# FlinkML/flink-parameter-server

Hardware: NVIDIA H100
Metric: matrix-factorization updates/sec (whole box, max over ranks) (higher is better)
Workload: dtype fp32

## Files before the change

flink-parameter-server_b200/models/mf/device.py:

```python
from __future__ import annotations

import math
import os
from typing import Iterable, Optional, Sequence, Tuple

import torch
import torch.distributed as dist

from ...errors import FactorIsNotANumberException
from ...ops import native
from ...utils.metrics import GLOBAL as METRICS
from ...runtime.device_stream import DevicePrefetcher
from ...store.replica_cache import ReplicaCache
from ...store.sharded_table import ShardedTable

ERR_SIGMOID = 0
ERR_PLAIN = 1

DEFAULT_DEVICE_PULL_LIMIT = 0

L2_TABLE_BYTES = 48 << 20
WINDOW_BUDGET = 256 << 20
WINDOW_BYTES_PER_ROW = 8 + 12
WINDOW_MAX_STRIDE = 128
# ... 89 lines not shown
                 output_ring=None, loss: str = "pointwise", regularization: float = 0.0,
                 step_window: Optional[int] = None, optimizer: str = "sgd",
                 negative_sampling: str = "uniform", margin: Optional[float] = None):
        self._pending = []
        self.step_window = 0
        check_negative_sampling(negative_sampling, negative_sample_rate)
        self.negative_sampling = negative_sampling
        if loss not in ("pointwise", "bpr", "warp"):
            raise ValueError(f"loss must be 'pointwise', 'bpr' or 'warp', got {loss!r}")
        self.loss, self.reg = loss, float(regularization)
        if loss == "pointwise" and self.reg != 0.0:
            raise ValueError("regularization is only supported with loss='bpr' or loss='warp'")
        self.margin = check_warp(loss, margin, optimizer=optimizer, negative_sampling=negative_sampling)
        if loss != "pointwise":
            if output_ring is not None:
                raise ValueError(f"the per-update output ring is not supported with loss={loss!r}")
            if kernel == "tma":
                raise ValueError(f"kernel='tma' is not supported with loss={loss!r}")
            if item_blocking:
                raise ValueError(f"item_blocking is not supported with loss={loss!r}")
            item_blocking = False
        self.device = torch.cuda.current_device() if device is None else int(device)
        self.cuda_device = torch.device("cuda", self.device)
        self.group = group
        ready = dist.is_available() and dist.is_initialized()
        self.world = dist.get_world_size(group) if ready else 1
        self.rank = dist.get_rank(group) if ready else 0
        if item_cache is None:
            item_cache = self.world > 1 and os.environ.get("FPS_ITEM_CACHE", "1") != "0"
        check_optimizer(optimizer, item_cache=bool(item_cache), output_ring=output_ring, kernel=kernel)
        self.optimizer = optimizer
        self.num_users, self.num_items, self.k = int(num_users), int(num_items), int(num_factors)
        self.lr = float(learning_rate)
        self.neg = int(negative_sample_rate)
        self.pull_limit = int(pull_limit)
        self.err_mode = int(err_mode)
        self.seed = int(seed)
        self.step_no = 0
        self.kernel = kernel
        self.credits = (torch.tensor([self.pull_limit, 0], dtype=torch.int32, device=self.cuda_device)
                        if self.pull_limit >= 32 and os.environ.get("FPS_STATIC_LIMITER", "0") != "1"
                        and loss == "pointwise" and optimizer == "sgd" else None)
        self.output_ring = output_ring
        with torch.cuda.device(self.device):
            self._items = ShardedTable(num_items, num_factors, partition="hash", group=group,
                                      device=self.device, init="uniform",
                                      init_range=(range_min, range_max), seed=seed * 2 + 1,
                                      track_touched=track_touched)
            n_local = -(-self.num_users // self.world)
            self._users = torch.empty((n_local, self._items.stride), dtype=torch.float32,
                                     device=self.cuda_device)
            native.init_rows(self._users, self.k, self.rank, self.world, native.PART_HASH, n_local,
                             seed * 2 + 2, range_min, range_max)
            self._stats = torch.zeros(STATS_SIZE[loss], dtype=torch.float32, device=self.cuda_device)
            self._user_acc = self._item_acc = None
            if optimizer == "adagrad":
                self._user_acc = torch.zeros(n_local, dtype=torch.float32, device=self.cuda_device)
                self._item_acc = self._items.row_accumulators()
            self._nan_flag = torch.zeros(1, dtype=torch.int32, device=self.cuda_device)
            self.user_memory = int(user_memory) if self.neg > 0 else 0
            if self.user_memory > 0:
                self.seen = torch.full((n_local, self.user_memory), -1, dtype=torch.int32,
                                       device=self.cuda_device)
                self.seen_pos = torch.zeros(n_local, dtype=torch.int32, device=self.cuda_device)
            self._registry = (native.seen_registry(self.num_items, self.cuda_device)
                              if negative_sampling == "seen" else None)
        self.item_cache = bool(item_cache)
        self.sync_every = max(1, int(sync_every))
        self.sync_interval_ms = sync_interval_ms
        self.flush_count, self.flush_require = flush_count, flush_require
        self._own_inplace = replica_own_inplace
        self.replica = (ReplicaCache(self._items, self.sync_every, sync_interval_ms,
                                     require=flush_require, flush_count=flush_count,
                                     own_inplace=replica_own_inplace)
                        if self.item_cache else None)
        row_bytes = self._items.stride * 4
        if item_blocking is None:
            item_blocking = ((self.world == 1 or self.item_cache) and self.num_items * row_bytes > (48 << 20)
                             and (self.neg == 0 or self.user_memory > 0 or negative_sampling == "seen")
                             and os.environ.get("FPS_ITEM_BLOCKING", "1") != "0")
        self.item_blocking = bool(item_blocking)
        block_bytes = int(os.environ.get("FPS_BLOCK_BYTES", block_bytes))
        self.l2_hints = self.item_blocking and os.environ.get("FPS_L2_HINTS", "0") == "1"
        per_bucket = max(1, int(block_bytes) // row_bytes)
        self.block_shift = max(0, per_bucket.bit_length() - 1)
        table_rows = self._items.rows_per_shard * self.world if self.item_cache else self.num_items
        self._table_rows = table_rows
        while -(-table_rows >> self.block_shift) > native.BUCKET_MAX:
            self.block_shift += 1
        self.block_buckets = max(1, -(-table_rows >> self.block_shift))
        if self.item_blocking:
            with torch.cuda.device(self.device):
                self._bucket_scratch = torch.zeros(2 * native.BUCKET_MAX, dtype=torch.int32,
                                                   device=self.cuda_device)
        self.step_window = step_window_size(step_window, world=self.world, item_cache=self.item_cache,
                                            loss=self.loss, table_rows=self.num_items, stride=self._items.stride,
                                            env=os.environ.get("FPS_STEP_WINDOW"), optimizer=optimizer)
        self._win = None
        self._win_phase_ns = None
        self._graph_capture = False
        self._per_launch = False
        self._items.barrier()

    @property
    def stats(self) -> torch.Tensor:
        self._drain()
        return self._stats

    @property
    def users(self) -> torch.Tensor:
        self._drain()
        return self._users

    @property
    def items(self) -> ShardedTable:
        self._drain()
        return self._items

    @property
    def nan_flag(self) -> torch.Tensor:
        self._drain()
        return self._nan_flag

    @property
    def accumulators(self) -> Optional[Tuple[torch.Tensor, torch.Tensor]]:
        self._drain()
        if self._item_acc is None:
            return None
        return self._user_acc, self._item_acc.local

    def _windowable(self, users, items, ratings) -> bool:
        if self.step_window < 2 or self._graph_capture or self._per_launch:
            return False
        packed = items is None
        return step_windowable(
            neg=self.neg, output_ring=self.output_ring, pull_limit=self.pull_limit, credits=self.credits,
            kernel=self.kernel, kernel_env=os.environ.get("FPS_MF_KERNEL", "reg"),
            reg_variant_env=os.environ.get("FPS_MF_REG_VARIANT"), l2_hints=self.l2_hints, packed=packed,
            dtypes=(users.dtype,) if packed else (users.dtype, items.dtype, ratings.dtype),
            n_records=users.numel(), table_rows=self.num_items, on_gpu=users.is_cuda,
            capturing=torch.cuda.is_current_stream_capturing())

    def _stage(self, users, items, ratings) -> None:
        if self._win is None:
            rows, w = self.num_items, self.step_window
            slot_bytes = -(-rows * 12 // 256) * 256
            with torch.cuda.device(self.device):
                dev = self.cuda_device
                self._win = {
                    "slot_bytes": slot_bytes,
                    "stage": torch.empty(w * slot_bytes, dtype=torch.uint8, device=dev),
                    "slots": torch.full((w, rows), -1, dtype=torch.int64, device=dev),
                    "user_bits": torch.zeros(-(-self._users.shape[0] // 32), dtype=torch.int32, device=dev),
                    "ctl": torch.zeros(2 * native.WINDOW_MAX, dtype=torch.int32, device=dev),
                    "slot_stats": torch.zeros((w, 2), dtype=torch.float32, device=dev),
                }
        j = len(self._pending)
        n = users.numel()
        sb = self._win["slot_bytes"]
        slot = self._win["stage"][j * sb:(j + 1) * sb]
        if items is None:
            slot[:8 * n].view(torch.int64).copy_(users.reshape(-1), non_blocking=True)
        else:
            ids = slot[:12 * n].view(torch.int32)
            ids[:n].copy_(users.reshape(-1), non_blocking=True)
            ids[n:2 * n].copy_(items.reshape(-1), non_blocking=True)
            ids[2 * n:].view(torch.float32).copy_(ratings.reshape(-1), non_blocking=True)
        self._pending.append((n, 1 if items is None else 0))
        self.step_no += 1
        METRICS.inc("mf_ratings", n)

    def _drain(self) -> int:
        n = len(self._pending)
        if n == 0:
            return 0
        counts, fmts = zip(*self._pending)
        self._pending = []
        w = self._win
        native.mf_window_drain(w["stage"], w["slot_bytes"], counts, fmts, self._users, self._items.local, self.lr,
                               self.err_mode, w["slots"], w["user_bits"], w["ctl"], self._stats, w["slot_stats"],
                               self._nan_flag, phase_ns=self._win_phase_ns)
        return n

    def flush(self) -> None:
        self._drain()
        if self.replica is not None:
            self.replica.flush()

    def step(self, users: torch.Tensor, items: Optional[torch.Tensor] = None,
             ratings: Optional[torch.Tensor] = None, negatives: Optional[torch.Tensor] = None) -> None:
        if self.loss == "pointwise" and negatives is None and self._windowable(users, items, ratings):
            self._stage(users, items, ratings)
            if len(self._pending) >= self.step_window:
                self._drain()
            return
        self._drain()
        check_negative_sampling(self.negative_sampling, self.neg, negatives)
        if self.loss != "pointwise":
            self._step_pairwise(users, items, ratings, negatives)
            return
        if negatives is not None:
            raise ValueError("negatives= needs loss='bpr' or loss='warp'")
        neg = self.neg
        if self.user_memory > 0 or self._registry is not None:
            users, items, ratings = self._sample_negatives(users, items, ratings)
            neg = 0
        n_records = users.numel()
        fed = False
        ring = self.output_ring
        out_args = ring.kernel_args() if ring is not None else None
        revisits = self.item_cache or n_records * (1 + neg) > self._table_rows
        if self.item_blocking and self.block_buckets > 1 and revisits:
            hashed = self.item_cache and self._items.mode == native.PART_HASH
            fed = hashed
            users, items, ratings = native.bucket_by_item(
                users, items, ratings, self.block_shift, self.block_buckets, self._bucket_scratch,
                num_shards=self.world if hashed else 1, rows_per_shard=self._items.rows_per_shard,
                pending=self.replica.pending if hashed else None)
        if self.item_cache:
            self.replica.after_step(n_records * (1 + neg), fed=fed)
            native.mf_sgd_fused(users, items, ratings, self._users, self.world, self.replica.table_c,
                                self.lr, err_mode=self.err_mode, neg_rate=neg,
                                num_items=self.num_items, seed=self.seed, step=self.step_no,
                                stats=self._stats, nan_flag=self._nan_flag,
                                max_inflight_rows=self.pull_limit, kernel="reg", l2_hints=self.l2_hints,
                                reserve_total=self.replica.reserve_total(), output=out_args,
                                credits=self.credits)
        else:
            native.mf_sgd_fused(users, items, ratings, self._users, self.world, self._items.table_c,
                                self.lr, err_mode=self.err_mode, neg_rate=neg,
                                num_items=self.num_items, seed=self.seed, step=self.step_no,
                                stats=self._stats, nan_flag=self._nan_flag,
                                max_inflight_rows=self.pull_limit, kernel=self.kernel,
                                l2_hints=self.l2_hints, output=out_args, credits=self.credits,
                                item_acc=self._item_acc.table_c if self._item_acc is not None else None,
                                user_acc=self._user_acc)
        if ring is not None:
            ring.after_kernel(users.numel() * (1 + neg))
        self.step_no += 1
        METRICS.inc("mf_ratings", users.numel())

    def _step_pairwise(self, users, items, ratings, negatives) -> None:
        if negatives is not None:
            if self.item_cache:
                raise ValueError("negatives= is not supported in the replica (item_cache) mode")
            n = int(negatives.shape[1]) if negatives.dim() == 2 else 0
        elif self.neg < 1:
            raise ValueError(f"loss={self.loss!r} needs negative_sample_rate >= 1 or explicit negatives=")
        elif self.user_memory > 0 or self._registry is not None:
            per = 1 + self.neg
            ou, oi, orat = self._sample_negatives(users, items, ratings)
            ou, oi = ou.view(-1, per), oi.view(-1, per)
            negatives = torch.where(ou[:, 1:] >= 0, oi[:, 1:], torch.full_like(oi[:, 1:], -1)).contiguous()
            users, items, ratings = ou[:, 0].contiguous(), oi[:, 0].contiguous(), orat.view(-1, per)[:, 0].contiguous()
            n = self.neg
        else:
            n = self.neg
        if self.output_ring is not None:
            raise ValueError(f"the per-update output ring is not supported with loss={self.loss!r}")
        n_pos = users.numel()
        cand, reserve = self._items.table_c, 0
        if self.item_cache:
            self.replica.after_step(n_pos * (n if self.loss == "bpr" else 1), fed=False)
            cand, reserve = self.replica.table_c, self.replica.reserve_total()
        if self.loss == "warp":
            native.mf_warp_fused(users, items, ratings, self._users, cand, self.lr, self.reg, margin=self.margin,
                                 rank_items=self.num_items, negatives=negatives, n_neg=n, num_items=self.num_items,
                                 seed=self.seed, step=self.step_no, anchor_div=self.world, stats=self._stats,
                                 nan_flag=self._nan_flag, max_inflight_rows=self.pull_limit, reserve_total=reserve)
            self.step_no += 1
            METRICS.inc("mf_ratings", n_pos)
            return
        native.mf_bpr_fused(users, items, ratings, self._users, cand, self.lr, self.reg, negatives=negatives,
                            n_neg=n, num_items=self.num_items, seed=self.seed, step=self.step_no,
                            anchor_div=self.world, stats=self._stats, nan_flag=self._nan_flag,
                            max_inflight_rows=self.pull_limit, reserve_total=reserve,
                            anchor_acc=self._user_acc,
                            cand_acc=self._item_acc.table_c if self._item_acc is not None else None)
        self.step_no += 1
        METRICS.inc("mf_ratings", n_pos)

    def _sample_negatives(self, users, items, ratings):
        memory = self.user_memory > 0
        if self._registry is not None:
            return native.neg_sample_seen(users, items, ratings, self.neg, self._registry,
                                          self.seen if memory else None, self.seen_pos if memory else None,
                                          self.world, seed=self.seed, step=self.step_no)
        return native.neg_sample(users, items, ratings, self.neg, self.num_items, self.seen, self.seen_pos,
                                 self.world, seed=self.seed, step=self.step_no)

    def seen_items(self) -> torch.Tensor:
        if self._registry is None:
            raise ValueError("seen_items() needs negative_sampling='seen'")
        order, count, _ = self._registry
        return order[:int(count.item())].to(torch.int64)

    def make_graph_step(self, batch_size: int, packed: bool = True):
        self._drain()
        dev = self.cuda_device
        if packed:
            static = (torch.zeros(batch_size, dtype=torch.int64, device=dev),)
        else:
            static = (torch.zeros(batch_size, dtype=torch.int32, device=dev),
                      torch.zeros(batch_size, dtype=torch.int32, device=dev),
                      torch.zeros(batch_size, dtype=torch.float32, device=dev))
        s = torch.cuda.Stream(device=dev)
        s.wait_stream(torch.cuda.current_stream(dev))
# ... 127 lines not shown
```

flink-parameter-server_b200/ops/csrc/fps_mf_window.cu:

```cuda
#include <cuda_fp16.h>
#include <cooperative_groups.h>
#include "fps_common.cuh"
#include "fps_mf_args.cuh"

namespace cg = cooperative_groups;

#define WIN_MAX 8
#define WIN_THREADS 256
#define WIN_EMPTY 0xFFFFFFFFFFFFFFFFull

struct WinArgs {
  const unsigned char* stage;
  long long slot_bytes;
  long long n[WIN_MAX];
  int fmt[WIN_MAX];
  int n_slots;
  int err_mode;
  float lr;
  int stride;
  float* user_table;
  float* item_table;
  long long rows;
  unsigned long long* slots;
  unsigned int* user_bits;
  long long bm_words;
  unsigned int* ctl;
  float* stats;
  float* slot_stats;
  int* nan_flag;
  unsigned long long* phase_ns;
};

__device__ __forceinline__ bool win_record(const WinArgs& a, int j, long long i, int& user, int& item,
                                           float& rating) {
  const unsigned char* base = a.stage + (long long)j * a.slot_bytes;
  if (a.fmt[j] == 1) {
    const unsigned long long rec = reinterpret_cast<const unsigned long long*>(base)[i];
    user = (int)(rec >> 38);
    item = (int)((rec >> 16) & 0x3FFFFFull);
    rating = __half2float(__ushort_as_half((unsigned short)(rec & 0xFFFFull)));
    return true;
  }
  const long long n = a.n[j];
  user = reinterpret_cast<const int*>(base)[i];
  item = reinterpret_cast<const int*>(base)[n + i];
  rating = reinterpret_cast<const float*>(base)[2 * n + i];
  return user >= 0;
}

__device__ __forceinline__ float win_add(float x, float y) {
  float z;
  asm("add.rn.ftz.f32 %0, %1, %2;" : "=f"(z) : "f"(x), "f"(y));
  return z;
}
__device__ __forceinline__ float4 win_add4(float4 x, float g, float4 y) {
  return make_float4(win_add(x.x, g * y.x), win_add(x.y, g * y.y), win_add(x.z, g * y.z), win_add(x.w, g * y.w));
}

__device__ __forceinline__ unsigned long long win_clock() {
  unsigned long long t;
  asm volatile("mov.u64 %0, %%globaltimer;" : "=l"(t));
  return t;
}
__device__ __forceinline__ void win_phase(const WinArgs& a, int k) {
  const unsigned long long t = win_clock();
  a.phase_ns[k] += t - a.phase_ns[3];
  a.phase_ns[3] = t;
  if (k == 1) a.phase_ns[2] += 1ull;
}

template <int G, int NS>
__device__ __forceinline__ void win_flush_stats(const WinArgs& a, float (&sq)[NS], float (&cnt)[NS], int nr,
                                                int slot0, float* sh) {
  const int lane = threadIdx.x & (G - 1);
  __syncthreads();
  if (threadIdx.x < 2 * WIN_MAX) sh[threadIdx.x] = 0.f;
  __syncthreads();
#pragma unroll
  for (int r = 0; r < WIN_MAX; ++r) {
    if (r < nr) {
      const bool mine = lane == r % G;
      float s = mine ? sq[r / G] : 0.f, c = mine ? cnt[r / G] : 0.f;
#pragma unroll
      for (int o = 16; o > 0; o >>= 1) {
        s += __shfl_xor_sync(0xffffffffu, s, o);
        c += __shfl_xor_sync(0xffffffffu, c, o);
      }
      if ((threadIdx.x & 31) == 0 && c > 0.f) {
        atomicAdd(sh + 2 * r, s);
        atomicAdd(sh + 2 * r + 1, c);
      }
    }
  }
#pragma unroll
  for (int i = 0; i < NS; ++i) sq[i] = cnt[i] = 0.f;
  __syncthreads();
  if (threadIdx.x < 2 * nr && sh[threadIdx.x] != 0.f)
    atomicAdd(a.slot_stats + 2 * slot0 + threadIdx.x, sh[threadIdx.x]);
}

template <int G, int VPL>
__device__ __forceinline__ void win_load(float4 (&x)[VPL], const float* row, int lane, int nvec, bool on) {
#pragma unroll
  for (int k = 0; k < VPL; ++k) {
    const int c = lane + k * G;
    x[k] = (on && c < nvec) ? *reinterpret_cast<const float4*>(row + 4 * c) : make_float4(0.f, 0.f, 0.f, 0.f);
  }
}
template <int G, int VPL>
__device__ __forceinline__ void win_store(float* row, const float4 (&x)[VPL], int lane, int nvec) {
#pragma unroll
  for (int k = 0; k < VPL; ++k) {
    const int c = lane + k * G;
    if (c < nvec) *reinterpret_cast<float4*>(row + 4 * c) = x[k];
  }
}
template <int G, int VPL>
__device__ __forceinline__ float win_dot(const float4 (&u)[VPL], const float4 (&v)[VPL]) {
  float d[VPL];
#pragma unroll
  for (int k = 0; k < VPL; ++k) {
    d[k] = 0.f;
    d[k] += fps_mf_dot4(u[k], v[k]);
  }
#pragma unroll
  for (int h = VPL / 2; h > 0; h >>= 1)
#pragma unroll
    for (int k = 0; k < h; ++k) d[k] += d[k + h];
  return fps_group_sum<G>(d[0]);
}

template <int LPR, int VPL, int P, int MINB>
__global__ void __launch_bounds__(WIN_THREADS, MINB) fps_mf_window_kernel(const __grid_constant__ WinArgs a) {
  static_assert(VPL >= 1 && VPL <= LPR && LPR % VPL == 0, "VPL must divide LPR");
  constexpr int G = LPR / VPL;
  __shared__ float sh[2 * WIN_MAX];
  cg::grid_group grid = cg::this_grid();
  const int lane = threadIdx.x & (G - 1);
  const int gtid = blockIdx.x * blockDim.x + threadIdx.x;
  const int gthreads = gridDim.x * blockDim.x;
  const int group = gtid / G;
  const int n_groups = gthreads / G;
  const int stride = a.stride;
  const int nvec = stride >> 2;
  constexpr int NS = G < WIN_MAX ? WIN_MAX / G : 1;
  constexpr int NE = NS;
  float sq[NS], cnt[NS];
#pragma unroll
  for (int i = 0; i < NS; ++i) sq[i] = cnt[i] = 0.f;
  bool bad = false;
  const bool timer = a.phase_ns != nullptr && blockIdx.x == 0 && threadIdx.x == 0;

  if (blockIdx.x == 0) {
    if (threadIdx.x < 2 * WIN_MAX) a.ctl[threadIdx.x] = 0u;
    if (threadIdx.x < 2 * a.n_slots) a.slot_stats[threadIdx.x] = 0.f;
  }
  if (timer) a.phase_ns[3] = win_clock();
  int start = 0, attempt = 0;
  while (start < a.n_slots) {
    for (long long w = gtid; w < a.bm_words; w += gthreads) a.user_bits[w] = 0u;
    grid.sync();
    int end = start;
    bool clashed = false;
    while (end < a.n_slots) {
      const int j = end;
      unsigned long long* t = a.slots + (long long)(j - start) * a.rows;
      bool clash = false;
      for (long long i = gtid; i < a.n[j]; i += gthreads) {
        int user, item;
        float rating;
        if (!win_record(a, j, i, user, item, rating)) continue;
        const unsigned long long e = ((unsigned long long)__float_as_uint(rating) << 32) | (unsigned int)user;
        clash |= atomicExch(t + item, e) != WIN_EMPTY;
        const unsigned int bit = 1u << (user & 31);
        clash |= (atomicOr(a.user_bits + (user >> 5), bit) & bit) != 0u;
      }
      if (clash) *reinterpret_cast<volatile unsigned int*>(a.ctl + attempt) = 1u;
      grid.sync();
      clashed = *reinterpret_cast<volatile unsigned int*>(a.ctl + attempt) != 0u;
      ++attempt;
      if (clashed) break;
      ++end;
    }
    if (timer) win_phase(a, 0);
    const int nrow = end - start;
    const int written = nrow + (clashed ? 1 : 0);
    if (nrow > 0) {
      unsigned long long nxt[NE];
#pragma unroll
      for (int m = 0; m < NE; ++m) {
        const int r = lane + m * G;
        nxt[m] = (group < a.rows && r < written) ? a.slots[(long long)r * a.rows + group] : WIN_EMPTY;
      }
      for (long long base = 0; base < a.rows; base += n_groups) {
        const long long item = base + group;
        const bool in = item < a.rows;
        float* vp = a.item_table + (in ? item : 0) * (long long)stride;
        float4 v[VPL];
#pragma unroll
        for (int k = 0; k < VPL; ++k) v[k] = make_float4(0.f, 0.f, 0.f, 0.f);
        bool any = false;
        bool loaded = false;
        unsigned long long mine[NE];
#pragma unroll
        for (int m = 0; m < NE; ++m) {
          const int r = lane + m * G;
          mine[m] = nxt[m];
          const long long it2 = item + n_groups;
          nxt[m] = (it2 < a.rows && r < written) ? a.slots[(long long)r * a.rows + it2] : WIN_EMPTY;
          if (mine[m] != WIN_EMPTY) a.slots[(long long)r * a.rows + item] = WIN_EMPTY;
        }
        const int src0 = (threadIdx.x & 31) & ~(G - 1);
#pragma unroll
        for (int c0 = 0; c0 < WIN_MAX; c0 += P) {
          if (c0 < nrow) {
            unsigned long long ent[P];
#pragma unroll
            for (int q = 0; q < P; ++q) {
              const int r = c0 + q;
              ent[q] = __shfl_sync(0xffffffffu, mine[(r / G) % NE], src0 + r % G);
              if (r >= nrow) ent[q] = WIN_EMPTY;
            }
            {
              bool chunk_any = false;
#pragma unroll
              for (int q = 0; q < P; ++q) chunk_any |= ent[q] != WIN_EMPTY;
              if (chunk_any && !loaded) win_load<G, VPL>(v, vp, lane, nvec, true);
              loaded |= chunk_any;
              any |= chunk_any;
              float4 u[P][VPL];
#pragma unroll
              for (int q = 0; q < P; ++q)
                win_load<G, VPL>(u[q], a.user_table + (long long)(unsigned int)ent[q] * stride, lane, nvec,
                                 ent[q] != WIN_EMPTY);
#pragma unroll
              for (int q = 0; q < P; ++q) {
                const int r = c0 + q;
                if (r < nrow) {
                  const float d = win_dot<G, VPL>(u[q], v);
                  const bool ok = ent[q] != WIN_EMPTY;
                  const float rating = __uint_as_float((unsigned int)(ent[q] >> 32));
                  const float resid = rating - d;
                  const float g = fps_mf_grad(a.err_mode, a.lr, rating, d, resid);
                  if (ok) {
                    if (!(fabsf(g) <= 3.0e38f)) bad = true;
                    if (lane == r % G) {
                      sq[r / G] += resid * resid;
                      cnt[r / G] += 1.f;
                    }
                    float4 nu[VPL];
#pragma unroll
                    for (int k = 0; k < VPL; ++k) {
                      nu[k] = win_add4(u[q][k], g, v[k]);
                      v[k] = win_add4(v[k], g, u[q][k]);
                    }
                    win_store<G, VPL>(a.user_table + (long long)(unsigned int)ent[q] * stride, nu, lane, nvec);
                  }
                }
              }
            }
          }
        }
        if (any) win_store<G, VPL>(vp, v, lane, nvec);
      }
      win_flush_stats<G, NS>(a, sq, cnt, nrow, start, sh);
    } else {
      const int j = start;
      unsigned long long* t = a.slots;
      for (long long base = 0; base < a.n[j]; base += n_groups) {
        const long long i = base + group;
        int user = 0, item = 0;
        float rating = 0.f;
        const bool ok = i < a.n[j] && win_record(a, j, i, user, item, rating);
        float* up = a.user_table + (long long)user * stride;
        float* vp = a.item_table + (long long)item * stride;
        float4 u[VPL], v[VPL];
#pragma unroll
        for (int k = 0; k < VPL; ++k) {
          const int c = lane + k * G;
          u[k] = v[k] = make_float4(0.f, 0.f, 0.f, 0.f);
          if (ok && c < nvec) {
            v[k] = fps_ld_row4(vp + 4 * c);
            u[k] = *reinterpret_cast<const float4*>(up + 4 * c);
          }
        }
        const float d = win_dot<G, VPL>(u, v);
        const float resid = rating - d;
        const float g = fps_mf_grad(a.err_mode, a.lr, rating, d, resid);
        if (ok) {
          if (!(fabsf(g) <= 3.0e38f)) bad = true;
          if (lane == 0) {
            sq[0] += resid * resid;
            cnt[0] += 1.f;
            t[item] = WIN_EMPTY;
          }
#pragma unroll
          for (int k = 0; k < VPL; ++k) {
            const int c = lane + k * G;
            if (c < nvec) {
              fps_red_add4(up + 4 * c, make_float4(g * v[k].x, g * v[k].y, g * v[k].z, g * v[k].w));
              fps_red_add4(vp + 4 * c, make_float4(g * u[k].x, g * u[k].y, g * u[k].z, g * u[k].w));
            }
          }
        }
      }
      win_flush_stats<G, NS>(a, sq, cnt, 1, start, sh);
      end = start + 1;
    }
    grid.sync();
    if (timer) win_phase(a, 1);
    start = end;
  }
  if (bad && a.nan_flag != nullptr) *a.nan_flag = 1;
  if (blockIdx.x == 0 && threadIdx.x == 0 && a.stats != nullptr) {
    float s = 0.f, c = 0.f;
    for (int j = 0; j < a.n_slots; ++j) {
      s += a.slot_stats[2 * j];
      c += a.slot_stats[2 * j + 1];
    }
    a.stats[0] += s;
    a.stats[1] += c;
  }
}

template <int LPR, int VPL, int P, int MINB>
static int launch_window(const WinArgs& a, int num_sms, cudaStream_t stream) {
  constexpr int V = VPL < LPR ? VPL : LPR;
  int occ = 0;
  cudaError_t e =
      cudaOccupancyMaxActiveBlocksPerMultiprocessor(&occ, fps_mf_window_kernel<LPR, V, P, MINB>, WIN_THREADS, 0);
  if (e != cudaSuccess) return (int)e;
  if (occ < 1) return -1402;
  const long long grid = (long long)num_sms * occ;
  WinArgs args = a;
  void* params[] = {&args};
  e = cudaLaunchCooperativeKernel((const void*)fps_mf_window_kernel<LPR, V, P, MINB>, dim3((unsigned)grid),
                                  dim3(WIN_THREADS), params, 0, stream);
  if (e != cudaSuccess) return (int)e;
  return (int)cudaGetLastError();
// ... 30 lines not shown
```

flink-parameter-server_b200/ops/native.py:

```python
from __future__ import annotations

import ctypes as C
import math
import os
import threading
from typing import Optional

import torch

from . import build as _build

FPS_MAX_SHARDS = 16
PART_HASH = 0
PART_RANGE = 1
PART_LUT = 2
LUT_OWNER_SHIFT = 40

_lib = None
_lib_lock = threading.Lock()
_launch_count = 0


class ShardTableC(C.Structure):

# ... 138 lines not shown
    _check(lib().fps_heap_free(C.c_void_p(ptr)), "heap_free")


def ipc_get_handle(ptr: int) -> bytes:
    buf = (C.c_ubyte * 64)()
    _check(lib().fps_ipc_get_handle(C.c_void_p(ptr), buf), "ipc_get_handle")
    return bytes(buf)


def ipc_open_handle(handle: bytes) -> int:
    buf = (C.c_ubyte * 64).from_buffer_copy(handle)
    out = C.c_void_p()
    _check(lib().fps_ipc_open_handle(buf, C.byref(out)), "ipc_open_handle")
    return int(out.value)


def ipc_close(ptr: int) -> None:
    _check(lib().fps_ipc_close(C.c_void_p(ptr)), "ipc_close")


def enable_peer(dev: int, peer: int) -> None:
    _check(lib().fps_enable_peer(int(dev), int(peer)), f"enable_peer({dev},{peer})")


class _RawCudaBuffer:

    def __init__(self, ptr: int, shape, typestr: str):
        self.__cuda_array_interface__ = {
            "shape": tuple(shape),
            "typestr": typestr,
            "data": (int(ptr), False),
            "version": 3,
            "strides": None,
        }


_TYPESTR = {torch.float32: "<f4", torch.int32: "<i4", torch.int64: "<i8", torch.uint8: "|u1",
            torch.float16: "<f2", torch.int16: "<i2"}


def tensor_from_ptr(ptr: int, shape, dtype: torch.dtype, device: int) -> torch.Tensor:
    if dtype == torch.bfloat16:
        t = torch.as_tensor(_RawCudaBuffer(ptr, shape, "<i2"), device=torch.device("cuda", device))
        return t.view(torch.bfloat16)
    return torch.as_tensor(_RawCudaBuffer(ptr, shape, _TYPESTR[dtype]),
                           device=torch.device("cuda", device))


def init_rows(rows: torch.Tensor, dim: int, shard: int, num_shards: int, mode: int, div: int,
              seed: int, lo: float, hi: float) -> None:
    _req(rows, "rows", torch.float32)
    n_rows, stride = rows.shape
    assert stride % 4 == 0
    _check(lib().fps_init_rows(C.c_void_p(rows.data_ptr()), C.c_longlong(n_rows), int(dim),
                               int(stride), int(shard), int(num_shards), int(mode),
                               C.c_longlong(div), C.c_ulonglong(seed & (2**64 - 1)),
                               C.c_float(lo), C.c_float(hi), _stream()), "init_rows")
    _bump()


def mf_sgd_fused(users: torch.Tensor, items: torch.Tensor, ratings: torch.Tensor,
                 user_table, user_div: int, item_tab: ShardTableC, lr: float,
                 err_mode: int = 0, neg_rate: int = 0, num_items: int = 0, seed: int = 0,
                 step: int = 0, stats: Optional[torch.Tensor] = None,
                 nan_flag: Optional[torch.Tensor] = None, max_inflight_rows: int = 0,
                 kernel: Optional[str] = None, push_tab: Optional[ShardTableC] = None,
                 l2_hints: bool = False, reserve_ctas: int = 0, reserve_total: int = 0,
                 progress: Optional[torch.Tensor] = None, output=None,
                 credits: Optional[torch.Tensor] = None, item_acc: Optional[ShardTableC] = None,
                 user_acc=None) -> None:
    _req(users, "users")
    user_sharded = isinstance(user_table, ShardTableC)
    if not user_sharded:
        _req(user_table, "user_table", torch.float32)
    packed = items is None
    if packed:
        if users.dtype != torch.int64:
            raise TypeError("packed rating records must be an int64 tensor (see pack_ratings)")
    else:
        _req(items, "items"); _req(ratings, "ratings", torch.float32)
        if users.dtype != items.dtype:
            raise TypeError("users and items must share an integer dtype")
    if (user_table.stride if user_sharded else user_table.shape[1]) != item_tab.stride:
        raise ValueError("user table stride must equal item table stride")
    a = MfArgsC()
    a.users = users.data_ptr()
    a.items = None if packed else items.data_ptr()
    a.ratings = None if packed else ratings.data_ptr()
    a.format = 1 if packed else 0
    a.n_pos = users.numel(); a.neg_rate = int(neg_rate); a.num_items = int(max(num_items, 1))
    a.seed = seed & (2**64 - 1); a.step = int(step)
    if user_sharded:
        a.user_table = None; a.user_tab = user_table; a.user_sharded = 1
    else:
        a.user_table = user_table.data_ptr(); a.user_sharded = 0
    a.user_div = int(user_div)
    a.user_shift = log2_or_neg(int(user_div))
    a.lr = float(lr); a.err_mode = int(err_mode)
    a.stats = stats.data_ptr() if stats is not None else None
    a.nan_flag = nan_flag.data_ptr() if nan_flag is not None else None
    a.item_tab = item_tab
    if push_tab is not None:
        a.push_tab = push_tab; a.use_push_tab = 1
    a.l2_hints = 1 if l2_hints else 0
    variant = kernel or os.environ.get("FPS_MF_KERNEL", "reg")
    if packed or push_tab is not None or l2_hints or output is not None or credits is not None:
        variant = "reg"
    a.progress = progress.data_ptr() if progress is not None else None
    if credits is not None:
        _req(credits, "credits", torch.int32)
        a.credits = credits.data_ptr()
    if output is not None:
        o_ids, o_vecs, o_staged, o_cap, o_every = output
        a.out_ids = o_ids.data_ptr(); a.out_vecs = o_vecs.data_ptr(); a.out_staged = o_staged.data_ptr()
        a.out_cap = int(o_cap); a.out_every = int(o_every)
    if item_acc is not None:
        if push_tab is not None or output is not None or credits is not None:
            raise ValueError("row-wise AdaGrad does not support push_tab, output or credits")
        if int(item_acc.stride) != 1:
            raise ValueError("item_acc must be a stride-1 accumulator table")
        a.item_acc = item_acc
        if user_sharded:
            if not isinstance(user_acc, ShardTableC) or int(user_acc.stride) != 1:
                raise ValueError("a sharded user table needs a stride-1 ShardTableC user_acc")
            a.user_acc_tab = user_acc
        else:
            if not torch.is_tensor(user_acc):
                raise ValueError("a worker-local user table needs a float32 user_acc tensor")
            _req(user_acc, "user_acc", torch.float32)
            if user_acc.numel() < user_table.shape[0]:
                raise ValueError("user_acc must hold one accumulator per user row")
            a.user_acc = user_acc.data_ptr()
        variant = "reg"
    elif user_acc is not None:
        raise ValueError("user_acc needs item_acc")
    lib().fps_set_mf_reserve(int(reserve_ctas))
    lib().fps_set_mf_reserve_total(int(reserve_total))
    rv = os.environ.get("FPS_MF_REG_VARIANT")
    if rv is not None:
        lib().fps_set_mf_reg_variant(int(rv))
    if variant == "tma":
        code = lib().fps_mf_sgd_tma(C.byref(a), _id_bytes(users), int(max_inflight_rows),
                                    sm_count(users.device.index), _stream())
        if code != -1002:
            _check(code, "mf_sgd_tma")
            _bump()
            return
    _check(lib().fps_mf_sgd_fused(C.byref(a), 4 if packed else _id_bytes(users), int(max_inflight_rows),
                                  sm_count(users.device.index), _stream()), "mf_sgd_fused")
    _bump()


WINDOW_MAX = 8


class WinArgsC(C.Structure):

    _fields_ = [
        ("stage", C.c_void_p), ("slot_bytes", C.c_longlong),
        ("n", C.c_longlong * WINDOW_MAX), ("fmt", C.c_int * WINDOW_MAX),
        ("n_slots", C.c_int), ("err_mode", C.c_int), ("lr", C.c_float), ("stride", C.c_int),
        ("user_table", C.c_void_p), ("item_table", C.c_void_p), ("rows", C.c_longlong),
        ("slots", C.c_void_p), ("user_bits", C.c_void_p), ("bm_words", C.c_longlong),
        ("ctl", C.c_void_p), ("stats", C.c_void_p), ("slot_stats", C.c_void_p), ("nan_flag", C.c_void_p),
        ("phase_ns", C.c_void_p),
    ]


def mf_window_drain(stage: torch.Tensor, slot_bytes: int, counts, formats, user_table: torch.Tensor,
                    item_table: torch.Tensor, lr: float, err_mode: int, slots: torch.Tensor,
                    user_bits: torch.Tensor, ctl: torch.Tensor, stats: torch.Tensor, slot_stats: torch.Tensor,
                    nan_flag: torch.Tensor, phase_ns: Optional[torch.Tensor] = None) -> None:
    n = len(counts)
    if not 0 < n <= WINDOW_MAX or len(formats) != n:
        raise ValueError(f"1..{WINDOW_MAX} staged micro-batches expected, got {n}")
    for t, name in ((stage, "stage"), (user_table, "user_table"), (item_table, "item_table"), (slots, "slots"),
                    (user_bits, "user_bits"), (ctl, "ctl"), (stats, "stats"), (slot_stats, "slot_stats"),
                    (nan_flag, "nan_flag")):
        _req(t, name)
    if user_table.shape[1] != item_table.shape[1]:
        raise ValueError("user table stride must equal item table stride")
    if user_bits.numel() * 32 < user_table.shape[0] or slots.numel() < n * item_table.shape[0]:
        raise ValueError("user bitmap or slot table too small")
    if slot_stats.numel() < 2 * n or ctl.numel() < 2 * WINDOW_MAX:
        raise ValueError("slot_stats / ctl too small")
    a = WinArgsC()
    a.stage = stage.data_ptr(); a.slot_bytes = int(slot_bytes)
    for j in range(n):
        a.n[j] = int(counts[j]); a.fmt[j] = int(formats[j])
    a.n_slots = n; a.err_mode = int(err_mode); a.lr = float(lr); a.stride = int(item_table.shape[1])
    a.user_table = user_table.data_ptr(); a.item_table = item_table.data_ptr(); a.rows = int(item_table.shape[0])
    a.slots = slots.data_ptr(); a.user_bits = user_bits.data_ptr(); a.bm_words = user_bits.numel()
    a.ctl = ctl.data_ptr(); a.stats = stats.data_ptr(); a.slot_stats = slot_stats.data_ptr()
    a.nan_flag = nan_flag.data_ptr()
    if phase_ns is not None:
        _req(phase_ns, "phase_ns", torch.int64)
        if phase_ns.numel() < 4:
            raise ValueError("phase_ns too small")
        a.phase_ns = phase_ns.data_ptr()
    rv = os.environ.get("FPS_MF_WINDOW_VARIANT")
    if rv is not None:
        lib().fps_set_mf_window_variant(int(rv))
    _check(lib().fps_mf_window_drain(C.byref(a), sm_count(stage.device.index), _stream()), "mf_window_drain")
    _bump()


class BprArgsC(C.Structure):

    _fields_ = [
        ("users", C.c_void_p), ("items", C.c_void_p), ("ratings", C.c_void_p), ("negatives", C.c_void_p),
        ("n_pos", C.c_longlong), ("n_neg", C.c_int), ("format", C.c_int),
        ("num_items", C.c_longlong), ("seed", C.c_ulonglong), ("step", C.c_ulonglong),
        ("lr", C.c_float), ("reg", C.c_float),
        ("anchor_table", C.c_void_p), ("anchor_div", C.c_int), ("anchor_shift", C.c_int),
        ("anchor_sharded", C.c_int), ("cand_sharded", C.c_int), ("anchor_tab", ShardTableC),
        ("cand_table", C.c_void_p), ("cand_div", C.c_int), ("cand_shift", C.c_int), ("cand_tab", ShardTableC),
        ("use_push_tab", C.c_int), ("stride", C.c_int), ("push_tab", ShardTableC),
        ("stats", C.c_void_p), ("nan_flag", C.c_void_p), ("reserve_total", C.c_int), ("pad_", C.c_int),
        ("anchor_acc_tab", ShardTableC), ("cand_acc", ShardTableC), ("anchor_acc", C.c_void_p),
        ("rank_items", C.c_longlong), ("margin", C.c_float), ("pad2_", C.c_int),
    ]


def _pairwise_args(users, items, ratings, anchor_table, cand_table, lr, reg, negatives, n_neg, num_items, seed,
                   step, anchor_div, cand_div, stats, n_stats, nan_flag, push_tab, reserve_total):
    _req(users, "users")
    packed = items is None
    if packed:
        if users.dtype != torch.int64:
            raise TypeError("packed rating records must be an int64 tensor (see pack_ratings)")
        id_dtype = torch.int32
    else:
        _req(items, "items"); _req(ratings, "ratings", torch.float32)
        if users.dtype != items.dtype:
            raise TypeError("users and items must share an integer dtype")
        if items.numel() != users.numel() or ratings.numel() != users.numel():
            raise ValueError("users, items and ratings must have the same length")
        id_dtype = users.dtype
    n_pos = users.numel()
    a = BprArgsC()
    strides = []
    for name, tab, div in (("anchor", anchor_table, anchor_div), ("cand", cand_table, cand_div)):
        if isinstance(tab, ShardTableC):
            setattr(a, f"{name}_tab", tab); setattr(a, f"{name}_sharded", 1)
            strides.append(int(tab.stride))
        else:
            _req(tab, f"{name}_table", torch.float32)
            setattr(a, f"{name}_table", tab.data_ptr())
            setattr(a, f"{name}_div", int(div)); setattr(a, f"{name}_shift", log2_or_neg(int(div)))
            strides.append(int(tab.shape[1]))
    if strides[0] != strides[1]:
        raise ValueError("anchor table stride must equal candidate table stride")
    a.stride = strides[0]
    if push_tab is not None:
        if not a.cand_sharded:
            raise ValueError("push_tab needs a ShardTable cand_table")
        if int(push_tab.stride) != a.stride:
            raise ValueError("push table stride must equal candidate table stride")
        a.push_tab = push_tab; a.use_push_tab = 1
    if negatives is not None:
        _req(negatives, "negatives", id_dtype)
        if negatives.dim() != 2 or negatives.shape[0] != n_pos:
            raise ValueError(f"negatives must be [{n_pos}, n]")
        a.negatives = negatives.data_ptr(); a.n_neg = int(negatives.shape[1])
    else:
        if int(n_neg) < 1:
            raise ValueError("n_neg must be >= 1 when negatives are sampled")
        a.n_neg = int(n_neg)
    if stats is not None:
        _req(stats, "stats", torch.float32)
        if stats.numel() < n_stats:
            raise ValueError(f"stats must hold {n_stats} floats")
        a.stats = stats.data_ptr()
    if nan_flag is not None:
        _req(nan_flag, "nan_flag", torch.int32)
        a.nan_flag = nan_flag.data_ptr()
    a.users = users.data_ptr()
    a.items = None if packed else items.data_ptr()
    a.ratings = None if packed else ratings.data_ptr()
    a.format = 1 if packed else 0
    a.n_pos = n_pos; a.num_items = int(max(num_items, 1))
    a.seed = seed & (2**64 - 1); a.step = int(step)
    a.lr = float(lr); a.reg = float(reg); a.reserve_total = int(reserve_total)
    return a, packed


def mf_bpr_fused(users: torch.Tensor, items: Optional[torch.Tensor], ratings: Optional[torch.Tensor],
                 anchor_table, cand_table, lr: float, reg: float = 0.0, *,
                 negatives: Optional[torch.Tensor] = None, n_neg: int = 1, num_items: int = 0,
                 seed: int = 0, step: int = 0, anchor_div: int = 1, cand_div: int = 1,
                 stats: Optional[torch.Tensor] = None, nan_flag: Optional[torch.Tensor] = None,
                 max_inflight_rows: int = 0, push_tab: Optional[ShardTableC] = None,
                 reserve_total: int = 0, anchor_acc=None, cand_acc: Optional[ShardTableC] = None) -> None:
    a, packed = _pairwise_args(users, items, ratings, anchor_table, cand_table, lr, reg, negatives, n_neg, num_items,
                               seed, step, anchor_div, cand_div, stats, 3, nan_flag, push_tab, reserve_total)
    if cand_acc is not None:
        if not a.cand_sharded or push_tab is not None:
            raise ValueError("row-wise AdaGrad needs a ShardTableC cand_table and no push_tab")
        if int(cand_acc.stride) != 1:
            raise ValueError("cand_acc must be a stride-1 accumulator table")
        a.cand_acc = cand_acc
        if a.anchor_sharded:
            if not isinstance(anchor_acc, ShardTableC) or int(anchor_acc.stride) != 1:
                raise ValueError("a sharded anchor table needs a stride-1 ShardTableC anchor_acc")
            a.anchor_acc_tab = anchor_acc
        else:
            if not torch.is_tensor(anchor_acc):
                raise ValueError("a worker-local anchor table needs a float32 anchor_acc tensor")
            _req(anchor_acc, "anchor_acc", torch.float32)
            if anchor_acc.numel() < anchor_table.shape[0]:
                raise ValueError("anchor_acc must hold one accumulator per anchor row")
            a.anchor_acc = anchor_acc.data_ptr()
    elif anchor_acc is not None:
        raise ValueError("anchor_acc needs cand_acc")
    _check(lib().fps_mf_bpr_fused(C.byref(a), 4 if packed else _id_bytes(users), int(max_inflight_rows),
                                  sm_count(users.device.index), _stream()), "mf_bpr_fused")
    _bump()


WARP_TRIAL_BLOCKS = (1, 2, 4, 8)


def mf_warp_fused(users: torch.Tensor, items: Optional[torch.Tensor], ratings: Optional[torch.Tensor],
                  anchor_table, cand_table, lr: float, reg: float = 0.0, *, margin: float = 1.0,
                  rank_items: int = 0, negatives: Optional[torch.Tensor] = None, n_neg: int = 1,
                  num_items: int = 0, seed: int = 0, step: int = 0, anchor_div: int = 1, cand_div: int = 1,
                  stats: Optional[torch.Tensor] = None, nan_flag: Optional[torch.Tensor] = None,
                  max_inflight_rows: int = 0, push_tab: Optional[ShardTableC] = None, reserve_total: int = 0,
                  trial_block: int = 0) -> None:
    if not math.isfinite(float(margin)):
        raise ValueError(f"margin must be finite, got {margin!r}")
    if int(trial_block) not in (0,) + WARP_TRIAL_BLOCKS:
        raise ValueError(f"trial_block must be 0 or one of {WARP_TRIAL_BLOCKS}, got {trial_block!r}")
    a, packed = _pairwise_args(users, items, ratings, anchor_table, cand_table, lr, reg, negatives, n_neg, num_items,
                               seed, step, anchor_div, cand_div, stats, 4, nan_flag, push_tab, reserve_total)
    a.margin = float(margin)
    a.rank_items = int(rank_items) if int(rank_items) > 0 else int(a.num_items)
# ... 765 lines not shown
```

Before: 3.297 billion.

## Scatter all window slots optimistically before one grid sync, fall back on clash

The window drain kernel used to scatter micro-batches one slot at a time with a grid-wide sync after each, so it could detect user or item clashes. It now scatters every remaining slot in one pass behind a single grid.sync and sets a shared once-flag if any clash appears. On a clash it clears the slot entries and the user bitmap and redoes the per-slot scatter with a sync per slot. This cuts grid barriers on the common clash-free path, but a clash now costs a wasted scatter, a cleanup pass and one extra control word.

```diff
diff --git a/flink-parameter-server_b200/models/mf/device.py b/flink-parameter-server_b200/models/mf/device.py
--- a/flink-parameter-server_b200/models/mf/device.py
+++ b/flink-parameter-server_b200/models/mf/device.py
@@ -265,7 +265,7 @@
                     "stage": torch.empty(w * slot_bytes, dtype=torch.uint8, device=dev),
                     "slots": torch.full((w, rows), -1, dtype=torch.int64, device=dev),
                     "user_bits": torch.zeros(-(-self._users.shape[0] // 32), dtype=torch.int32, device=dev),
-                    "ctl": torch.zeros(2 * native.WINDOW_MAX, dtype=torch.int32, device=dev),
+                    "ctl": torch.zeros(native.WINDOW_CTL_WORDS, dtype=torch.int32, device=dev),
                     "slot_stats": torch.zeros((w, 2), dtype=torch.float32, device=dev),
                 }
         j = len(self._pending)
diff --git a/flink-parameter-server_b200/ops/csrc/fps_mf_window.cu b/flink-parameter-server_b200/ops/csrc/fps_mf_window.cu
--- a/flink-parameter-server_b200/ops/csrc/fps_mf_window.cu
+++ b/flink-parameter-server_b200/ops/csrc/fps_mf_window.cu
@@ -48,6 +48,23 @@
   return user >= 0;
 }
 
+__device__ __forceinline__ volatile unsigned int* win_once(const WinArgs& a) { return a.ctl + 2 * WIN_MAX; }
+
+__device__ __noinline__ bool win_scatter(const WinArgs& a, int j, int start, int gtid, int gthreads) {
+  unsigned long long* t = a.slots + (long long)(j - start) * a.rows;
+  bool clash = false;
+  for (long long i = gtid; i < a.n[j]; i += gthreads) {
+    int user, item;
+    float rating;
+    if (!win_record(a, j, i, user, item, rating)) continue;
+    const unsigned long long e = ((unsigned long long)__float_as_uint(rating) << 32) | (unsigned int)user;
+    clash |= atomicExch(t + item, e) != WIN_EMPTY;
+    const unsigned int bit = 1u << (user & 31);
+    clash |= (atomicOr(a.user_bits + (user >> 5), bit) & bit) != 0u;
+  }
+  return clash;
+}
+
 __device__ __forceinline__ float win_add(float x, float y) {
   float z;
   asm("add.rn.ftz.f32 %0, %1, %2;" : "=f"(z) : "f"(x), "f"(y));
@@ -152,39 +169,47 @@
   const bool timer = a.phase_ns != nullptr && blockIdx.x == 0 && threadIdx.x == 0;
 
   if (blockIdx.x == 0) {
-    if (threadIdx.x < 2 * WIN_MAX) a.ctl[threadIdx.x] = 0u;
+    if (threadIdx.x <= 2 * WIN_MAX) a.ctl[threadIdx.x] = 0u;
     if (threadIdx.x < 2 * a.n_slots) a.slot_stats[threadIdx.x] = 0.f;
   }
   if (timer) a.phase_ns[3] = win_clock();
+  for (long long w = gtid; w < a.bm_words; w += gthreads) a.user_bits[w] = 0u;
+  grid.sync();
   int start = 0, attempt = 0;
   while (start < a.n_slots) {
-    for (long long w = gtid; w < a.bm_words; w += gthreads) a.user_bits[w] = 0u;
+    bool clash = false;
+    for (int j = start; j < a.n_slots; ++j) clash |= win_scatter(a, j, start, gtid, gthreads);
+    if (clash) *win_once(a) = 1u;
     grid.sync();
-    int end = start;
+    int end = a.n_slots;
     bool clashed = false;
-    while (end < a.n_slots) {
-      const int j = end;
-      unsigned long long* t = a.slots + (long long)(j - start) * a.rows;
-      bool clash = false;
-      for (long long i = gtid; i < a.n[j]; i += gthreads) {
-        int user, item;
-        float rating;
-        if (!win_record(a, j, i, user, item, rating)) continue;
-        const unsigned long long e = ((unsigned long long)__float_as_uint(rating) << 32) | (unsigned int)user;
-        clash |= atomicExch(t + item, e) != WIN_EMPTY;
-        const unsigned int bit = 1u << (user & 31);
-        clash |= (atomicOr(a.user_bits + (user >> 5), bit) & bit) != 0u;
-      }
-      if (clash) *reinterpret_cast<volatile unsigned int*>(a.ctl + attempt) = 1u;
+    if (*win_once(a) != 0u) {
+      for (int j = start; j < a.n_slots; ++j) {
+        unsigned long long* t = a.slots + (long long)(j - start) * a.rows;
+        for (long long i = gtid; i < a.n[j]; i += gthreads) {
+          int user, item;
+          float rating;
+          if (win_record(a, j, i, user, item, rating)) t[item] = WIN_EMPTY;
+        }
+      }
+      for (long long w = gtid; w < a.bm_words; w += gthreads) a.user_bits[w] = 0u;
       grid.sync();
-      clashed = *reinterpret_cast<volatile unsigned int*>(a.ctl + attempt) != 0u;
-      ++attempt;
-      if (clashed) break;
-      ++end;
+      if (blockIdx.x == 0 && threadIdx.x == 0) *win_once(a) = 0u;
+      end = start;
+      while (end < a.n_slots) {
+        if (win_scatter(a, end, start, gtid, gthreads))
+          *reinterpret_cast<volatile unsigned int*>(a.ctl + attempt) = 1u;
+        grid.sync();
+        clashed = *reinterpret_cast<volatile unsigned int*>(a.ctl + attempt) != 0u;
+        ++attempt;
+        if (clashed) break;
+        ++end;
+      }
     }
     if (timer) win_phase(a, 0);
     const int nrow = end - start;
     const int written = nrow + (clashed ? 1 : 0);
+    for (long long w = gtid; w < a.bm_words; w += gthreads) a.user_bits[w] = 0u;
     if (nrow > 0) {
       unsigned long long nxt[NE];
 #pragma unroll
diff --git a/flink-parameter-server_b200/ops/native.py b/flink-parameter-server_b200/ops/native.py
--- a/flink-parameter-server_b200/ops/native.py
+++ b/flink-parameter-server_b200/ops/native.py
@@ -314,6 +314,7 @@
 
 
 WINDOW_MAX = 8
+WINDOW_CTL_WORDS = 2 * WINDOW_MAX + 1
 
 
 class WinArgsC(C.Structure):
@@ -344,7 +345,7 @@
         raise ValueError("user table stride must equal item table stride")
     if user_bits.numel() * 32 < user_table.shape[0] or slots.numel() < n * item_table.shape[0]:
         raise ValueError("user bitmap or slot table too small")
-    if slot_stats.numel() < 2 * n or ctl.numel() < 2 * WINDOW_MAX:
+    if slot_stats.numel() < 2 * n or ctl.numel() < WINDOW_CTL_WORDS:
         raise ValueError("slot_stats / ctl too small")
     a = WinArgsC()
     a.stage = stage.data_ptr(); a.slot_bytes = int(slot_bytes)
```

New measurement: 3.331 billion (median of 6 runs). Within noise of the previous version (+1.0%).
